# KKKSQJ/DeepLearning

Hardware: NVIDIA H100
Metric: images/sec (ResNet-50 training step) (higher is better)
Workload: dtype bf16

## Files before the change

deeplearning_b200/csrc/abi_conv.cu:

```cuda
#include <string.h>
#include "../../include/b200cls.h"
#include "conv_gemm.cuh"
#include "conv1x1_stream.cuh"
#include "conv_tap64.cuh"
#include "host_utils.h"
#include "wgrad_gemm.cuh"

using namespace b200;

namespace {

constexpr uint32_t kFwdDescLbo = 16, kFwdDescSbo = 1024;
constexpr uint32_t kWgDescLbo = 8192, kWgDescSbo = 1024, kWgDescKstep = 2048;

struct Box3 {
  int b1, b2, b3;
};

Box3 choose_box(long long d1, long long d2, long long d3, int P) {
  Box3 best{P, 1, 1};
  double best_cost = -1;
  for (int b1 = 1; b1 <= P; b1 <<= 1) {
    for (int b2 = 1; b1 * b2 <= P; b2 <<= 1) {
      const int b3 = P / (b1 * b2);
// ... 245 lines not shown
  B200_CHECK_CUDA(launch_pdl(conv_tap64_kernel<kStats>, dim3(grid), dim3(384), kTap64SmemBytes, st, q));
  B200_LAUNCHED();
  return OK;
}

template <int BLOCK_N>
int launch_conv_gemm(const ConvGemmParams& p, cudaStream_t st) {
  const int tiles = p.tiles1 * p.tiles2 * p.tiles3 * p.n_tiles;
  const int grid = conv_grid(tiles, p.n_tiles, p.stats != nullptr);
  B200_REQUIRE(grid > 0, "conv_gemm: %d channel blocks exceed the SM count (BN statistics need grid %% n_tiles == 0)", p.n_tiles);
  ConvGemmParams q = p;
  q.desc_lbo = kFwdDescLbo;
  q.desc_sbo = kFwdDescSbo;
  if constexpr (BLOCK_N == 64) {
    if (tap64_ok(p)) return p.stats != nullptr ? launch_tap64<true>(q, grid, st) : launch_tap64<false>(q, grid, st);
  }
  switch (epilogue_flags(p)) {
#define B200_EPI_CASE(F) \
  case (F):              \
    return launch_conv_gemm_epi<BLOCK_N, (F)>(q, grid, st);
    B200_EPI_LIST(B200_EPI_CASE)
#undef B200_EPI_CASE
    default:
      return launch_conv_gemm_epi<BLOCK_N, kEpiGeneric>(q, grid, st);
  }
}


bool stream_ok(long long pixels, int K, int N) {
  return (K == 64 || K == 128 || K == 256) && N % 256 == 0 && pixels % 128 == 0 && pixels / 128 < (1LL << 30);
}
int stream_grid(long long pixels, int N) {
  const int n_tiles = N / 256;
  const long long items = pixels / 128 * n_tiles;
  int grid = items < device_sm_count() ? static_cast<int>(items) : device_sm_count();
  return grid / n_tiles * n_tiles;
}

template <int KB, int MODE>
int launch_stream(const StreamParams& q, int grid, cudaStream_t st) {
  using Cfg = StreamCfg<KB, MODE>;
  static bool configured = false;
  if (!configured) {
    B200_CHECK_CUDA(cudaFuncSetAttribute(conv1x1_stream_kernel<KB, MODE>, cudaFuncAttributeMaxDynamicSharedMemorySize,
                                         Cfg::SMEM_BYTES));
    configured = true;
  }
  B200_CHECK_CUDA(launch_pdl(conv1x1_stream_kernel<KB, MODE>, dim3(grid), dim3(Cfg::THREADS), Cfg::SMEM_BYTES, st, q));
  B200_LAUNCHED();
  return OK;
}

int run_stream(int mode, const void* a, const void* w, void* out, const void* res, const void* mask, const float* scale,
               const float* shift, float* stats, long long pixels, int K, int N, cudaStream_t st) {
  StreamParams q;
  memset(&q, 0, sizeof(q));
  int rc;
  if ((rc = encode_matrix(&q.a_map, a, K, pixels, 128))) return rc;
  if ((rc = encode_matrix(&q.b_map, w, K, N, 256))) return rc;
  if ((rc = encode_matrix(&q.out_map, out, N, pixels, 16))) return rc;
  if (res != nullptr && (rc = encode_matrix(&q.res_map, res, N, pixels, 16))) return rc;
  if (mask != nullptr && (rc = encode_matrix(&q.mask_map, mask, N, pixels, 16))) return rc;
  q.m_tiles = static_cast<int>(pixels / 128);
  q.n_tiles = N / 256;
  q.N = N;
  q.scale = scale, q.shift = shift, q.stats = stats;
  const int grid = stream_grid(pixels, N);
  if (mode == kStreamAffine)
    return K == 64 ? launch_stream<1, kStreamAffine>(q, grid, st)
                   : (K == 128 ? launch_stream<2, kStreamAffine>(q, grid, st) : launch_stream<4, kStreamAffine>(q, grid, st));
  if (mode == kStreamBnRelu)
    return K == 64 ? launch_stream<1, kStreamBnRelu>(q, grid, st)
                   : (K == 128 ? launch_stream<2, kStreamBnRelu>(q, grid, st) : launch_stream<4, kStreamBnRelu>(q, grid, st));
  return K == 64 ? launch_stream<1, kStreamMask>(q, grid, st)
                 : (K == 128 ? launch_stream<2, kStreamMask>(q, grid, st) : launch_stream<4, kStreamMask>(q, grid, st));
}

int dispatch_conv_gemm(ConvGemmParams& p, int N, cudaStream_t st) {
  if (N <= 64) return launch_conv_gemm<64>(p, st);
  return launch_conv_gemm<128>(p, st);
}
int block_n_for(int N) { return N <= 64 ? 64 : 128; }

template <int BLOCK_NG, bool kGrouped = false>
int launch_wgrad(const WgradParams& p, cudaStream_t st) {
  using Cfg = WgradCfg<BLOCK_NG>;
  static bool configured = false;
  if (!configured) {
    if constexpr (kGrouped) {
      B200_CHECK_CUDA(cudaFuncSetAttribute(wgrad_gemm_kernel<BLOCK_NG, false, true>,
                                           cudaFuncAttributeMaxDynamicSharedMemorySize, Cfg::SMEM_BYTES));
    } else {
      B200_CHECK_CUDA(cudaFuncSetAttribute(wgrad_gemm_kernel<BLOCK_NG, false>, cudaFuncAttributeMaxDynamicSharedMemorySize,
                                           Cfg::SMEM_BYTES));
      B200_CHECK_CUDA(cudaFuncSetAttribute(wgrad_gemm_kernel<BLOCK_NG, true>, cudaFuncAttributeMaxDynamicSharedMemorySize,
                                           Cfg::SMEM_BYTES));
    }
    configured = true;
  }
  const int items = p.mg_tiles * p.ng_tiles * p.num_taps * p.splits;
  const int grid = items < device_sm_count() ? items : device_sm_count();
  WgradParams q = p;
  q.desc_lbo = kWgDescLbo;
  q.desc_sbo = kWgDescSbo;
  q.desc_kstep = kWgDescKstep;
  if constexpr (kGrouped)
    B200_CHECK_CUDA(launch_pdl(wgrad_gemm_kernel<BLOCK_NG, false, true>, dim3(grid), dim3(kWgradThreads), Cfg::SMEM_BYTES, st, q));
  else if (q.bias_partial != nullptr)
    B200_CHECK_CUDA(launch_pdl(wgrad_gemm_kernel<BLOCK_NG, true>, dim3(grid), dim3(kWgradThreads), Cfg::SMEM_BYTES, st, q));
  else
    B200_CHECK_CUDA(launch_pdl(wgrad_gemm_kernel<BLOCK_NG, false>, dim3(grid), dim3(kWgradThreads), Cfg::SMEM_BYTES, st, q));
  B200_LAUNCHED();
  return OK;
}

int launch_wgrad_reduce(const float* partial, float* dw, int splits, int Cout, int Cin, int taps, int accumulate,
                        cudaStream_t st, const float* bias_partial = nullptr, float* bias_out = nullptr) {
  const long long total = static_cast<long long>(Cout) * Cin * taps;
  if (Cin % 8 == 0 && (reinterpret_cast<uintptr_t>(partial) & 15) == 0) {
    int chunk = taps == 1 ? 256 : 64;
    while (chunk > 16 && chunk / 2 >= Cin) chunk /= 2;
    while (chunk > 16 && static_cast<long long>(Cout) * ((Cin + chunk - 1) / chunk) < 2ll * device_sm_count()) chunk /= 2;
    const int SL = splits < 8 ? splits : 8;
    const size_t smem = static_cast<size_t>(SL) * taps * chunk * sizeof(float);
    if (smem <= 48 * 1024 && Cout <= 65535 * 32) {
      dim3 grid(Cout, (Cin + chunk - 1) / chunk);
      B200_CHECK_CUDA(launch_pdl(wgrad_reduce_rows_kernel, dim3(grid), dim3(256), smem, st, partial, dw, splits, Cout, Cin, taps, chunk, SL, accumulate, bias_partial, bias_out));
      return OK;
    }
  }
  int blocks = static_cast<int>((total + 255) / 256);
  if (blocks > device_sm_count() * 8) blocks = device_sm_count() * 8;
  B200_CHECK_CUDA(launch_pdl(wgrad_reduce_flat_kernel, dim3(blocks), dim3(256), 0, st, partial, dw, splits, Cout, Cin, taps, accumulate, bias_partial, bias_out));
  return OK;
}

struct WgradPlan {
  int block_ng, mg_tiles, ng_tiles, taps;
  int merge_atoms;
  Box3 box;
  int tiles1, tiles2, tiles3, kb_total, splits, kb_per_split;
  int Ho, Wo;
};

WgradPlan plan_wgrad_geom(long long d1, long long d2, long long d3, int Cin, int Cout, int taps, bool grouped = false) {
  WgradPlan pl;
  pl.taps = taps;
  pl.Ho = static_cast<int>(d2), pl.Wo = static_cast<int>(d1);
  pl.block_ng = Cin <= 64 ? 64 : (((Cin + 255) / 256) * 48 < ((Cin + 127) / 128) * 32 ? 256 : 128);
  pl.mg_tiles = (Cout + 127) / 128;
  pl.ng_tiles = (Cin + pl.block_ng - 1) / pl.block_ng;
  pl.merge_atoms = 0;
  if (grouped) {
    pl.block_ng = 384;
    pl.ng_tiles = 1;
  } else if (Cin == 64 && taps > 1 && (taps % 4 == 0 || taps % 3 == 0)) {
    pl.merge_atoms = 1;
    pl.block_ng = taps % 4 == 0 ? 256 : 192;
    pl.ng_tiles = taps * 64 / pl.block_ng;
  }
  pl.box = choose_box(d1, d2, d3, 64);
  pl.tiles1 = static_cast<int>((d1 + pl.box.b1 - 1) / pl.box.b1);
  pl.tiles2 = static_cast<int>((d2 + pl.box.b2 - 1) / pl.box.b2);
  pl.tiles3 = static_cast<int>((d3 + pl.box.b3 - 1) / pl.box.b3);
  pl.kb_total = pl.tiles1 * pl.tiles2 * pl.tiles3;
  const int items_per_split = pl.mg_tiles * pl.ng_tiles * (pl.merge_atoms ? 1 : (grouped ? pl.taps / 3 : pl.taps));
  const int sms = device_sm_count();
  const double t_kb = pl.block_ng >= 256 ? 0.45 : (pl.block_ng == 192 ? 0.36 : (pl.block_ng == 128 ? 0.30 : 0.25));
  const double part_us = static_cast<double>(Cout) * Cin * taps * 4.0 * 2.0 / 3.0e6;
  const int max_splits = pl.kb_total / 4 > 0 ? pl.kb_total / 4 : 1;
  int splits = 1;
  double best = 1e30;
  for (int s = 1; s <= max_splits; ++s) {
    const int kps = (pl.kb_total + s - 1) / s;
    const int s2 = (pl.kb_total + kps - 1) / kps;
    if (s2 != s) continue;
    const int waves = (items_per_split * s + sms - 1) / sms;
    if (waves > 2 && items_per_split <= sms) continue;
    const double cost = waves * (kps * t_kb + 2.0) + s * part_us;
    if (cost < best) best = cost, splits = s;
    if (waves > 4 && s > 8) break;
  }
  pl.kb_per_split = (pl.kb_total + splits - 1) / splits;
  pl.splits = (pl.kb_total + pl.kb_per_split - 1) / pl.kb_per_split;
  return pl;
}

WgradPlan plan_wgrad(int B, int H, int W, int Cin, int Cout, int ksize, int stride, bool grouped = false) {
  const Dims3 d = out_dims(B, H, W, ksize, stride);
  WgradPlan pl = plan_wgrad_geom(d.d1, d.d2, d.d3, Cin, Cout, ksize * ksize, grouped);
  pl.Ho = out_dim(H, ksize, stride), pl.Wo = out_dim(W, ksize, stride);
  return pl;
}

size_t wgrad_bytes(const WgradPlan& pl, int Cout, int Cin) {
  return static_cast<size_t>(pl.splits) * Cout * pl.taps * Cin * sizeof(float);
}

WgradParams wgrad_params(const WgradPlan& pl, int Cout, int Cin, void* workspace) {
  WgradParams p;
  memset(&p, 0, sizeof(p));
  p.num_taps = pl.merge_atoms ? 1 : pl.taps;
  p.merge_atoms = pl.merge_atoms;
  p.n_cols = pl.merge_atoms ? pl.taps * Cin : Cin;
  p.Cout = Cout, p.Cin = Cin;
  p.mg_tiles = pl.mg_tiles, p.ng_tiles = pl.ng_tiles;
  p.tiles1 = pl.tiles1, p.tiles2 = pl.tiles2, p.tiles3 = pl.tiles3;
  p.box1 = pl.box.b1, p.box2 = pl.box.b2, p.box3 = pl.box.b3;
  p.splits = pl.splits, p.kb_per_split = pl.kb_per_split, p.kb_total = pl.kb_total;
  p.ld_partial = static_cast<long long>(pl.taps) * Cin;
  p.partial = static_cast<float*>(workspace);
  return p;
}

int setup_wgrad_maps(WgradParams& p, const WgradPlan& pl, const void* dy, const void* x, int B, int H, int W, int Cin,
                     int Cout, int ksize, int stride) {
  int rc;
  if ((rc = encode_view(&p.dy_map, act_view(dy, B, pl.Ho, pl.Wo, Cout, ksize == 1 && stride == 1), pl.box))) return rc;
  return encode_taps(p, p.x_maps, x, B, H, W, Cin, ksize, stride, pl.box);
}

View stem_s2d_view(const void* z, int B, int Ho, int Wo) {
  const int Hz = Ho + 3, Wz = Wo + 3;
  View v;
  v.base = z;
  v.dims[0] = 64, v.dims[1] = Wo, v.dims[2] = Hz, v.dims[3] = B;
  v.strides[0] = 1, v.strides[1] = 16, v.strides[2] = static_cast<uint64_t>(Wz) * 16;
  v.strides[3] = static_cast<uint64_t>(Hz) * Wz * 16;
  return v;
}

}

extern "C" {

static int fwd_stats_rows(int B, int H, int W, int Cout, int ksize, int stride, int BN) {
  const Dims3 d = out_dims(B, H, W, ksize, stride);
  const Box3 bx = choose_box(d.d1, d.d2, d.d3, 128);
  const long long m_tiles = ((d.d1 + bx.b1 - 1) / bx.b1) * ((d.d2 + bx.b2 - 1) / bx.b2) * ((d.d3 + bx.b3 - 1) / bx.b3);
  const int n_tiles = (Cout + BN - 1) / BN;
  const long long tiles = m_tiles * n_tiles;
  const int grid = conv_grid(tiles > (1 << 30) ? (1 << 30) : static_cast<int>(tiles), n_tiles, true);
  return grid / n_tiles * (BN == 64 ? 8 : 4);
}

int b200_conv2d_fwd_stats_rows(int B, int H, int W, int Cout, int ksize, int stride) {
  return fwd_stats_rows(B, H, W, Cout, ksize, stride, block_n_for(Cout));
}

static int conv_fwd(const void* x, const void* w, void* y, int B, int H, int W, int Cin, int Cout, int ksize, int stride,
                    float* stats, const float* bias, int act, const void* residual, float* out_f32, long long ld_out,
                    const float* bn_scale, const float* bn_shift, int y_f32, int Cg, void* stream) {
  B200_REQUIRE(ksize == 1 || ksize == 3 || (ksize == 2 && stride == 2), "conv2d_fwd: ksize %d / stride %d unsupported", ksize, stride);
  B200_REQUIRE(stride == 1 || stride == 2, "conv2d_fwd: stride %d unsupported (1 or 2)", stride);
  B200_REQUIRE(Cin % 8 == 0 && Cout % 8 == 0, "conv2d_fwd: Cin=%d / Cout=%d must be multiples of 8", Cin, Cout);
  B200_REQUIRE(B > 0 && H > 0 && W > 0, "conv2d_fwd: empty input");
  B200_REQUIRE(stride == 1 || (H >= 2 && W >= 2), "conv2d_fwd: stride-2 needs H,W >= 2");
  B200_REQUIRE(out_f32 == nullptr || (ksize == 1 && stride == 1), "conv2d_fwd: fp32 output only for 1x1/s1");
  B200_REQUIRE((bn_scale == nullptr) == (bn_shift == nullptr), "conv2d_fwd: bn_scale and bn_shift go together");
  B200_REQUIRE(bn_scale == nullptr || (Cout % 64 == 0 && bias == nullptr && stats == nullptr && out_f32 == nullptr && act <= 1 && !y_f32),
               "conv2d_fwd + folded BN: Cout=%d must be a multiple of 64, no bias / statistics / fp32 output", Cout);
  cudaStream_t st = static_cast<cudaStream_t>(stream);
  const int Ho = out_dim(H, ksize, stride), Wo = out_dim(W, ksize, stride);
  ConvGemmParams p;
  memset(&p, 0, sizeof(p));
  int rc;
  View dv = act_view(y, B, Ho, Wo, Cout, ksize == 1 && stride == 1);
  if (out_f32 != nullptr) dv.base = nullptr;
// ... 115 lines not shown
int b200_conv2d_dgrad(const void* dy, const void* wd, void* dx, int B, int H, int W, int Cin, int Cout, int ksize,
                      int stride, const void* residual, const b200_bn_mask_t* bn_mask, void* stream) {
  return conv_dgrad(dy, wd, dx, B, H, W, Cin, Cout, ksize, stride, residual, bn_mask, 0, stream);
}

int b200_gemm_ex(const b200_view_t* a, const b200_view_t* out, const b200_gemm_args_t* g, void* stream) {
  B200_REQUIRE(a != nullptr && out != nullptr && g != nullptr && g->w != nullptr, "gemm_ex: null argument");
  B200_REQUIRE(g->N % 8 == 0 && g->K % 8 == 0, "gemm_ex: N=%d / K=%d must be multiples of 8", g->N, g->K);
  for (int i = 0; i < 3; ++i)
    B200_REQUIRE(a->dim[i] == out->dim[i] && a->dim[i] > 0, "gemm_ex: a/out pixel extents differ in dim %d", i);
  B200_REQUIRE(!(g->aux_out != nullptr && g->out_f32), "gemm_ex: aux_out needs a bf16 primary output");
  B200_REQUIRE(!(g->stats != nullptr && g->out_f32), "gemm_ex: stats need a bf16 output");
  auto to_view = [](const b200_view_t* v, int C) {
    View r;
    r.base = v->base;
    r.dims[0] = C;
    r.strides[0] = 1;
    for (int i = 0; i < 3; ++i) {
      r.dims[i + 1] = static_cast<uint64_t>(v->dim[i]);
      r.strides[i + 1] = static_cast<uint64_t>(v->stride[i]);
    }
    return r;
  };
  ConvGemmParams p;
  memset(&p, 0, sizeof(p));
  int rc;
  View dv = to_view(out, g->N);
  View auxv;
  if (g->aux_out) auxv = to_view(g->aux_out, g->N);
  if ((rc = setup_output(p, dv, g->N, g->out_f32, g->aux_out ? &auxv : nullptr))) return rc;
  const Box3 bx = box_of(p);
  if ((rc = encode_view(&p.a_maps[0], to_view(a, g->K), bx))) return rc;
  for (int i = 1; i < 4; ++i) p.a_maps[i] = p.a_maps[0];
  p.num_taps = 1;
  p.k_per_tap = g->K;
  p.k_blocks_per_tap = (g->K + 63) / 64;
  if ((rc = encode_matrix(&p.b_map, g->w, g->K, g->N, block_n_for(g->N)))) return rc;
  p.stats = g->stats;
  p.bias = g->bias;
  p.colscale = g->colscale;
  p.act = g->act;
  if (g->residual) {
    p.residual = g->residual->base;
    p.res_f32 = g->residual_f32;
    p.rs1 = g->residual->stride[0], p.rs2 = g->residual->stride[1], p.rs3 = g->residual->stride[2];
  }
  if (g->rowscale != nullptr) {
    B200_REQUIRE(g->rows_per_sample > 0, "gemm_ex: rowscale needs rows_per_sample > 0");
    p.rowscale = g->rowscale;
    p.rows_per_sample = g->rows_per_sample;
  }
  if (g->act == B200_ACT_GELU_GRAD) {
    B200_REQUIRE(g->aux_in != nullptr, "gemm_ex: B200_ACT_GELU_GRAD needs aux_in");
    p.aux_in = static_cast<const __nv_bfloat16*>(g->aux_in->base);
    p.as1 = g->aux_in->stride[0], p.as2 = g->aux_in->stride[1], p.as3 = g->aux_in->stride[2];
  }
  return dispatch_conv_gemm(p, g->N, static_cast<cudaStream_t>(stream));
}

int b200_conv2d_wgrad_splits(int B, int H, int W, int Cin, int Cout, int ksize, int stride) {
  return plan_wgrad(B, H, W, Cin, Cout, ksize, stride).splits;
}

size_t b200_conv2d_wgrad_workspace_bytes(int B, int H, int W, int Cin, int Cout, int ksize, int stride) {
  return wgrad_bytes(plan_wgrad(B, H, W, Cin, Cout, ksize, stride), Cout, Cin);
}

int b200_conv2d_wgrad(const void* dy, const void* x, float* dw, void* workspace, size_t workspace_bytes, int B, int H,
                      int W, int Cin, int Cout, int ksize, int stride, int accumulate, float* bias_partial, float* bias_out,
                      void* stream) {
  B200_REQUIRE(ksize == 1 || ksize == 3 || (ksize == 2 && stride == 2), "conv2d_wgrad: ksize %d / stride %d unsupported", ksize, stride);
  B200_REQUIRE(stride == 1 || stride == 2, "conv2d_wgrad: stride %d unsupported", stride);
  B200_REQUIRE(Cin % 8 == 0 && Cout % 8 == 0, "conv2d_wgrad: Cin=%d / Cout=%d must be multiples of 8", Cin, Cout);
  B200_REQUIRE(bias_out == nullptr || bias_partial != nullptr, "conv2d_wgrad: bias_out needs bias_partial");
  cudaStream_t st = static_cast<cudaStream_t>(stream);
  const WgradPlan pl = plan_wgrad(B, H, W, Cin, Cout, ksize, stride);
  const size_t need = wgrad_bytes(pl, Cout, Cin);
  B200_REQUIRE(workspace != nullptr && workspace_bytes >= need, "conv2d_wgrad: workspace too small (%zu < %zu)",
               workspace_bytes, need);
  WgradParams p = wgrad_params(pl, Cout, Cin, workspace);
  p.bias_partial = bias_partial;
  int rc;
  if ((rc = setup_wgrad_maps(p, pl, dy, x, B, H, W, Cin, Cout, ksize, stride))) return rc;
  if (pl.block_ng == 64)
    rc = launch_wgrad<64>(p, st);
  else if (pl.block_ng == 128)
    rc = launch_wgrad<128>(p, st);
  else if (pl.block_ng == 192)
    rc = launch_wgrad<192>(p, st);
  else
    rc = launch_wgrad<256>(p, st);
  if (rc) return rc;
  if ((rc = launch_wgrad_reduce(p.partial, dw, pl.splits, Cout, Cin, pl.taps, accumulate, st, bias_partial, bias_out))) return rc;
  B200_LAUNCHED();
  return OK;
}

int b200_stem_s2d_conv_fwd(const void* z, const void* w, void* y, float* stats, int B, int Ho, int Wo, void* stream) {
  B200_REQUIRE(B > 0 && Ho > 0 && Wo > 0, "stem_s2d_conv_fwd: empty output");
  cudaStream_t st = static_cast<cudaStream_t>(stream);
  const int Cout = 64;
  ConvGemmParams p;
  memset(&p, 0, sizeof(p));
  int rc;
  if ((rc = setup_output(p, make_view(y, B, Ho, Wo, Cout, 1, 0, 0), Cout, 0, nullptr))) return rc;
  const Box3 bx = box_of(p);
  p.k_per_tap = 64;
  p.k_blocks_per_tap = 1;
  p.num_taps = 4;
  if ((rc = encode_view(&p.a_maps[0], stem_s2d_view(z, B, Ho, Wo), bx))) return rc;
  for (int i = 1; i < 4; ++i) p.a_maps[i] = p.a_maps[0];
  for (int ky = 0; ky < 4; ++ky) {
    p.tap_map[ky] = 0, p.tap_o1[ky] = 0, p.tap_o2[ky] = static_cast<int8_t>(ky), p.tap_w[ky] = static_cast<int8_t>(ky);
  }
  if ((rc = encode_matrix(&p.b_map, w, 256, Cout, 64))) return rc;
  p.stats = stats;
  return dispatch_conv_gemm(p, Cout, st);
}

size_t b200_stem_s2d_conv_wgrad_workspace_bytes(int B, int Ho, int Wo) {
  return wgrad_bytes(plan_wgrad_geom(Wo, Ho, B, 64, 64, 4), 64, 64);
}

int b200_stem_s2d_conv_wgrad(const void* dy, const void* z, float* g, void* workspace, size_t workspace_bytes, int B, int Ho,
                             int Wo, void* stream) {
  cudaStream_t st = static_cast<cudaStream_t>(stream);
  const int Cout = 64, Cin = 64, taps = 4;
  const WgradPlan pl = plan_wgrad_geom(Wo, Ho, B, Cin, Cout, taps);
  const size_t need = wgrad_bytes(pl, Cout, Cin);
  B200_REQUIRE(workspace != nullptr && workspace_bytes >= need, "stem_s2d_conv_wgrad: workspace too small (%zu < %zu)",
               workspace_bytes, need);
  WgradParams p = wgrad_params(pl, Cout, Cin, workspace);
  int rc;
  if ((rc = encode_view(&p.dy_map, make_view(dy, B, Ho, Wo, Cout, 1, 0, 0), pl.box))) return rc;
  if ((rc = encode_view(&p.x_maps[0], stem_s2d_view(z, B, Ho, Wo), pl.box))) return rc;
  for (int i = 1; i < 4; ++i) p.x_maps[i] = p.x_maps[0];
  for (int ky = 0; ky < 4; ++ky) p.tap_map[ky] = 0, p.tap_o1[ky] = 0, p.tap_o2[ky] = static_cast<int8_t>(ky);
  if ((rc = launch_wgrad<256>(p, st))) return rc;
  if ((rc = launch_wgrad_reduce(p.partial, g, pl.splits, Cout, Cin, taps, 0, st))) return rc;
  B200_LAUNCHED();
  return OK;
}


int b200_conv1x1_bn_act_fwd(const void* x, const void* w, const float* scale, const float* shift, const void* residual,
                            void* y, long long pixels, int Cin, int Cout, int relu, void* stream) {
  B200_REQUIRE(pixels > 0 && Cin % 64 == 0 && Cout % 64 == 0, "conv1x1_bn_act_fwd: Cin=%d / Cout=%d must be multiples of 64", Cin, Cout);
  B200_REQUIRE(scale != nullptr && shift != nullptr && residual != nullptr && relu == 1,
               "conv1x1_bn_act_fwd: implemented for relu(bn(conv) + residual)");
  if (stream_ok(pixels, Cin, Cout))
    return run_stream(kStreamBnRelu, x, w, y, residual, nullptr, scale, shift, nullptr, pixels, Cin, Cout,
                      static_cast<cudaStream_t>(stream));
  ConvGemmParams p;
  memset(&p, 0, sizeof(p));
  int rc;
  View dv = make_flat_view(y, pixels, Cout);
  if ((rc = setup_output(p, dv, Cout, 0, nullptr))) return rc;
  const Box3 bx = box_of(p);
  p.k_per_tap = Cin;
  p.k_blocks_per_tap = Cin / 64;
  p.num_taps = 1;
  if ((rc = encode_view(&p.a_maps[0], make_flat_view(x, pixels, Cin), bx))) return rc;
  for (int i = 1; i < 4; ++i) p.a_maps[i] = p.a_maps[0];
  if ((rc = encode_matrix(&p.b_map, w, Cin, Cout, block_n_for(Cout)))) return rc;
  p.affine = 1;
  p.colscale = scale;
  p.bias = shift;
  p.act = 1;
  p.residual = residual;
  p.rs1 = static_cast<long long>(dv.strides[1]);
  p.rs2 = static_cast<long long>(dv.strides[2]);
  p.rs3 = static_cast<long long>(dv.strides[3]);
  return dispatch_conv_gemm(p, Cout, static_cast<cudaStream_t>(stream));
}

int b200_conv1x1_bn_fwd(const void* x, const void* w, const float* scale, const float* shift, void* y, long long pixels,
                        int Cin, int Cout, void* stream) {
  B200_REQUIRE(pixels > 0 && Cin % 64 == 0 && Cout % 64 == 0, "conv1x1_bn_fwd: Cin=%d / Cout=%d must be multiples of 64", Cin, Cout);
  B200_REQUIRE(scale != nullptr && shift != nullptr, "conv1x1_bn_fwd: scale / shift required");
  if (stream_ok(pixels, Cin, Cout))
    return run_stream(kStreamAffine, x, w, y, nullptr, nullptr, scale, shift, nullptr, pixels, Cin, Cout,
                      static_cast<cudaStream_t>(stream));
  return conv_fwd(x, w, y, 1, 1, static_cast<int>(pixels), Cin, Cout, 1, 1, nullptr, nullptr, 0, nullptr, nullptr, 0, scale,
                  shift, 0, 0, stream);
}

int b200_conv1x1_dgrad_masked_stats_rows(long long pixels, int Cin, int Cout) {
  if (stream_ok(pixels, Cout, Cin)) return stream_grid(pixels, Cin) / (Cin / 256) * 4;
  return b200_conv2d_fwd_stats_rows(1, 1, static_cast<int>(pixels), Cin, 1, 1);
}

int b200_conv1x1_dgrad_masked(const void* dy, const void* wd, void* dx, long long pixels, int Cin, int Cout,
                              const void* residual, const void* mask_src, float* stats, void* stream) {
  B200_REQUIRE(pixels > 0 && Cin % 64 == 0 && Cout % 64 == 0, "conv1x1_dgrad_masked: Cin=%d / Cout=%d must be multiples of 64", Cin, Cout);
  B200_REQUIRE(residual != nullptr && mask_src != nullptr && stats != nullptr, "conv1x1_dgrad_masked: residual, mask and stats are required");
  if (stream_ok(pixels, Cout, Cin))
    return run_stream(kStreamMask, dy, wd, dx, residual, mask_src, nullptr, nullptr, stats, pixels, Cout, Cin,
                      static_cast<cudaStream_t>(stream));
  ConvGemmParams p;
  memset(&p, 0, sizeof(p));
  int rc;
  View dv = make_flat_view(dx, pixels, Cin);
  if ((rc = setup_output(p, dv, Cin, 0, nullptr))) return rc;
  const Box3 bx = box_of(p);
  p.k_per_tap = Cout;
  p.k_blocks_per_tap = Cout / 64;
  p.num_taps = 1;
  if ((rc = encode_view(&p.a_maps[0], make_flat_view(dy, pixels, Cout), bx))) return rc;
  for (int i = 1; i < 4; ++i) p.a_maps[i] = p.a_maps[0];
  if ((rc = encode_matrix(&p.b_map, wd, Cout, Cin, block_n_for(Cin)))) return rc;
  p.residual = residual;
  p.rs1 = static_cast<long long>(dv.strides[1]);
  p.rs2 = static_cast<long long>(dv.strides[2]);
  p.rs3 = static_cast<long long>(dv.strides[3]);
  p.mask_in = static_cast<const __nv_bfloat16*>(mask_src);
  p.ms1 = p.rs1, p.ms2 = p.rs2, p.ms3 = p.rs3;
  p.stats = stats;
  return dispatch_conv_gemm(p, Cin, static_cast<cudaStream_t>(stream));
}

int b200_gemm_dual(const void* a0, int K0, const void* a1, int K1, const void* wcat, const float* bias, void* out,
// ... 90 lines not shown
```

deeplearning_b200/csrc/wgrad_gemm.cuh:

```cuda
#pragma once
#include "common.cuh"
#include "conv_gemm.cuh"
#include "conv1x1_stream.cuh"

namespace b200 {

struct alignas(64) WgradParams {
  CUtensorMap dy_map;
  CUtensorMap x_maps[4];
  int num_taps;
  int merge_atoms;
  int n_cols;
  int Cout, Cin;
  int mg_tiles, ng_tiles;
  int tiles1, tiles2, tiles3;
  int box1, box2, box3;
  int splits, kb_per_split, kb_total;
  long long ld_partial;
  int8_t tap_map[kMaxTaps];
  int8_t tap_o1[kMaxTaps];
  int8_t tap_o2[kMaxTaps];
  float* partial;
  uint32_t desc_lbo, desc_sbo, desc_kstep;
  float* bias_partial;
};

template <int BLOCK_NG>
struct WgradCfg {
  static constexpr int BLOCK_K = 64;
  static constexpr int A_BYTES = 2 * 64 * 128;
  static constexpr int B_BYTES = (BLOCK_NG / 64) * 64 * 128;
  static constexpr int STAGE_BYTES = A_BYTES + B_BYTES;
  static constexpr int STAGES = BLOCK_NG == 384 ? 3 : (BLOCK_NG == 256 ? 4 : (BLOCK_NG == 192 ? 5 : (BLOCK_NG == 128 ? 6 : 8)));
  static constexpr int BAR_BYTES = 256;
  static constexpr int SMEM_BYTES = STAGES * STAGE_BYTES + BAR_BYTES + 1024;
  static_assert(SMEM_BYTES <= 227 * 1024, "shared memory of one H100 block");
};
constexpr int kWgradThreads = 384;

template <int BLOCK_NG, bool kBias = false, bool kGrouped = false>
__global__ void __launch_bounds__(kWgradThreads, 1) wgrad_gemm_kernel(const __grid_constant__ WgradParams p) {
  static_assert(!kGrouped || (BLOCK_NG == 384 && !kBias), "grouped mode: two warpgroups x three 64-column taps");
  using Cfg = WgradCfg<BLOCK_NG>;
  constexpr int NW = kGrouped ? BLOCK_NG / 2 : BLOCK_NG;
  constexpr int STAGES = Cfg::STAGES;
  extern __shared__ uint8_t smem_raw[];
  uint8_t* smem = reinterpret_cast<uint8_t*>((reinterpret_cast<uintptr_t>(smem_raw) + 1023) & ~uintptr_t(1023));
  uint64_t* bars = reinterpret_cast<uint64_t*>(smem + STAGES * Cfg::STAGE_BYTES);
  uint64_t* full_bar = bars;
  uint64_t* empty_bar = bars + STAGES;
  __shared__ float bias_red[2][16][64];

  const int warp_idx = threadIdx.x >> 5;
  const int lane = threadIdx.x & 31;
  const int items_per_split = p.mg_tiles * p.ng_tiles * p.num_taps;
  const int num_items = items_per_split * p.splits;

  if (warp_idx == 0 && lane == 0) {
    tma_prefetch_desc(&p.dy_map);
    for (int i = 0; i < 4; ++i) tma_prefetch_desc(&p.x_maps[i]);
    for (int i = 0; i < STAGES; ++i) {
      mbar_init(&full_bar[i], 1);
      mbar_init(&empty_bar[i], kBias ? 8 : 2);
    }
    fence_mbar_init();
  }
  __syncthreads();
  pdl_wait();

  if (warp_idx < 4) {
    setmaxnreg_dec<40>();
    if (warp_idx == 0 && lane == 0) {
      int stage = 0;
      uint32_t phase = 0;
      for (int item = blockIdx.x; item < num_items; item += gridDim.x) {
        const int split = item / items_per_split;
        int r = item - split * items_per_split;
        const int tap = r % p.num_taps;
        r /= p.num_taps;
        const int ng = r % p.ng_tiles;
        const int mg = r / p.ng_tiles;
        const int kb0 = split * p.kb_per_split;
        const int kb1 = min(p.kb_total, kb0 + p.kb_per_split);
        const CUtensorMap* xm[BLOCK_NG / 64];
        int ch0[BLOCK_NG / 64], o1[BLOCK_NG / 64], o2[BLOCK_NG / 64];
#pragma unroll
        for (int j = 0; j < BLOCK_NG / 64; ++j) {
          int tp = tap, ca = ng * (BLOCK_NG / 64) + j;
          if constexpr (kGrouped) {
            tp = tap * 3 + j % 3;
            ca = mg * 2 + j / 3;
          } else if (p.merge_atoms) {
            tp = ca / p.merge_atoms;
            ca -= tp * p.merge_atoms;
          }
          xm[j] = &p.x_maps[p.tap_map[tp]];
          ch0[j] = ca * 64;
          o1[j] = p.tap_o1[tp], o2[j] = p.tap_o2[tp];
        }
        for (int kb = kb0; kb < kb1; ++kb) {
          const int t1 = kb % p.tiles1;
          const int t2 = (kb / p.tiles1) % p.tiles2;
          const int t3 = kb / (p.tiles1 * p.tiles2);
          const int c1 = t1 * p.box1, c2 = t2 * p.box2, c3 = t3 * p.box3;
          mbar_wait(&empty_bar[stage], phase ^ 1);
          uint8_t* a_dst = smem + stage * Cfg::STAGE_BYTES;
          uint8_t* b_dst = a_dst + Cfg::A_BYTES;
          mbar_expect_tx(&full_bar[stage], Cfg::STAGE_BYTES);
          tma_load_4d(a_dst, &p.dy_map, &full_bar[stage], mg * 128, c1, c2, c3);
          tma_load_4d(a_dst + 8192, &p.dy_map, &full_bar[stage], mg * 128 + 64, c1, c2, c3);
#pragma unroll
          for (int j = 0; j < BLOCK_NG / 64; ++j)
            tma_load_4d(b_dst + j * 8192, xm[j], &full_bar[stage], ch0[j], c1 + o1[j], c2 + o2[j], c3);
          if (++stage == STAGES) {
            stage = 0;
            phase ^= 1;
          }
        }
      }
    }
  } else {
    setmaxnreg_inc<232>();
    const int wg = (warp_idx >> 2) - 1;
    const bool leader = (threadIdx.x & 127) == 0;
    const uint64_t desc_a0 = make_smem_desc_sw128(smem_u32(smem) + wg * 8192, p.desc_lbo, p.desc_sbo);
    const uint64_t desc_b0 =
        make_smem_desc_sw128(smem_u32(smem) + Cfg::A_BYTES + (kGrouped ? wg * NW * 128 : 0), p.desc_lbo, p.desc_sbo);
    const uint64_t kstep = p.desc_kstep >> 4;
    const int t = threadIdx.x & 127;
    const int frow = 64 * wg + 16 * (t >> 5) + ((t & 31) >> 2);
    const int fcol = 2 * (t & 3);
    int stage = 0;
    uint32_t phase = 0;
    for (int item = blockIdx.x; item < num_items; item += gridDim.x) {
      const int split = item / items_per_split;
      int r = item - split * items_per_split;
      const int tap = r % p.num_taps;
      r /= p.num_taps;
      const int ng = r % p.ng_tiles;
      const int mg = r / p.ng_tiles;
      const int kb0 = split * p.kb_per_split;
      const int kb1 = min(p.kb_total, kb0 + p.kb_per_split);
      const bool summed = kBias && ng == 0 && tap == 0;
      const int cc = t & 7, rg = t >> 3;
      float bsum[8] = {0.f, 0.f, 0.f, 0.f, 0.f, 0.f, 0.f, 0.f};
      float acc[NW / 2];
#pragma unroll
      for (int i = 0; i < NW / 2; ++i) acc[i] = 0.f;
      int prev = -1;
      for (int kb = kb0; kb < kb1; ++kb) {
        mbar_wait(&full_bar[stage], phase);
        wgmma_fence();
        const uint64_t soff = static_cast<uint64_t>(stage) * (Cfg::STAGE_BYTES >> 4);
        const uint64_t da = desc_a0 + soff, db = desc_b0 + soff;
#pragma unroll
        for (int k = 0; k < 4; ++k) Wgmma<NW, 1, 1>::mma(acc, da + k * kstep, db + k * kstep, 1u);
        wgmma_commit();
        if (summed) {
          const uint32_t base = smem_u32(smem + stage * Cfg::STAGE_BYTES) + wg * 8192;
#pragma unroll
          for (int i = 0; i < 4; ++i) {
            const int r = rg * 4 + i;
            float f[8];
            unpack8(lds128(base + r * 128 + ((static_cast<uint32_t>(cc) ^ static_cast<uint32_t>(r & 7)) << 4)), f);
#pragma unroll
            for (int j = 0; j < 8; ++j) bsum[j] += f[j];
          }
        }
        wgmma_wait<1>();
        if constexpr (kBias) {
          __syncwarp();
          if (prev >= 0 && lane == 0) mbar_arrive(&empty_bar[prev]);
        } else {
          if (prev >= 0 && leader) mbar_arrive(&empty_bar[prev]);
        }
        prev = stage;
        if (++stage == STAGES) {
          stage = 0;
          phase ^= 1;
        }
      }
      wgmma_wait<0>();
      wgmma_reg_fence(acc);
      if constexpr (kBias) {
        __syncwarp();
        if (lane == 0) mbar_arrive(&empty_bar[prev]);
      } else {
        if (leader) mbar_arrive(&empty_bar[prev]);
      }
      if (summed) {
        named_bar_sync(1 + wg, 128);
#pragma unroll
        for (int j = 0; j < 8; ++j) bias_red[wg][rg][cc * 8 + j] = bsum[j];
        named_bar_sync(1 + wg, 128);
        if (t < 64) {
          float tot = 0.f;
#pragma unroll
          for (int g2 = 0; g2 < 16; ++g2) tot += bias_red[wg][g2][t];
          const int cout = mg * 128 + wg * 64 + t;
          if (cout < p.Cout) {
            p.bias_partial[(static_cast<long long>(split) * 2) * p.Cout + cout] = tot;
            p.bias_partial[(static_cast<long long>(split) * 2 + 1) * p.Cout + cout] = 0.f;
          }
        }
      }
      const int ncol = p.n_cols - ng * BLOCK_NG;
#pragma unroll
      for (int h = 0; h < 2; ++h) {
        const int cout = mg * 128 + frow + 8 * h;
        if (cout < p.Cout) {
          float* out_row = p.partial + (static_cast<long long>(split) * p.Cout + cout) * p.ld_partial +
                           static_cast<long long>(tap) * p.Cin + ng * BLOCK_NG;
#pragma unroll
          for (int j = 0; j < NW / 8; ++j)
            if (8 * j + fcol < ncol)
              *reinterpret_cast<float2*>(out_row + 8 * j + fcol) = make_float2(acc[4 * j + 2 * h], acc[4 * j + 2 * h + 1]);
        }
      }
    }
  }
}

__global__ void __launch_bounds__(256) wgrad_reduce_rows_kernel(const float* __restrict__ partial, float* __restrict__ grad,
                                                                int splits, int Cout, int Cin, int taps, int chunk, int SL,
                                                                int accumulate, const float* __restrict__ bias_partial,
                                                                float* __restrict__ bias_out) {
  pdl_wait();
  extern __shared__ float4 rows_sm4[];
  const int cout = blockIdx.x;
  if (bias_out != nullptr && blockIdx.y == 0 && threadIdx.x == 0) {
    float s = 0.f;
    for (int k = 0; k < splits; ++k) s += bias_partial[static_cast<long long>(k) * 2 * Cout + cout];
    bias_out[cout] = s;
  }
  const int c0 = blockIdx.y * chunk;
  const int cw = min(chunk, Cin - c0);
  const int vpt = cw >> 2;
  const int nvec = taps * vpt;
  const long long slice4 = static_cast<long long>(Cout) * taps * Cin / 4;
  const float4* row4 = reinterpret_cast<const float4*>(partial + static_cast<long long>(cout) * taps * Cin + c0);
  const int cin4 = Cin >> 2;
  for (int w = threadIdx.x; w < nvec * SL; w += blockDim.x) {
    const int sl = w / nvec;
    const int v = w - sl * nvec;
    const int tap = v / vpt;
    const int cv = v - tap * vpt;
    const float4* src = row4 + tap * cin4 + cv;
    float4 a = make_float4(0.f, 0.f, 0.f, 0.f), b = a;
    int k = sl;
    for (; k + SL < splits; k += 2 * SL) {
      const float4 x = __ldcs(src + k * slice4);
      const float4 y = __ldcs(src + (k + SL) * slice4);
      a.x += x.x, a.y += x.y, a.z += x.z, a.w += x.w;
      b.x += y.x, b.y += y.y, b.z += y.z, b.w += y.w;
    }
    if (k < splits) {
      const float4 x = __ldcs(src + k * slice4);
      a.x += x.x, a.y += x.y, a.z += x.z, a.w += x.w;
    }
    rows_sm4[w] = make_float4(a.x + b.x, a.y + b.y, a.z + b.z, a.w + b.w);
  }
  __syncthreads();
  const float* sm = reinterpret_cast<const float*>(rows_sm4);
  float* out = grad + (static_cast<long long>(cout) * Cin + c0) * taps;
  for (int e = threadIdx.x; e < cw * taps; e += blockDim.x) {
    const int cin = e / taps;
    const int tap = e - cin * taps;
    float s = 0.f;
    for (int sl = 0; sl < SL; ++sl) s += sm[(sl * nvec) * 4 + tap * cw + cin];
    out[e] = accumulate ? out[e] + s : s;
  }
}

__global__ void wgrad_reduce_flat_kernel(const float* __restrict__ partial, float* __restrict__ grad, int splits, int Cout,
                                    int Cin, int taps, int accumulate, const float* __restrict__ bias_partial,
                                    float* __restrict__ bias_out) {
  pdl_wait();
  const long long total = static_cast<long long>(Cout) * Cin * taps;
  const long long slice = total;
  if (bias_out != nullptr) {
    for (int cout = blockIdx.x * blockDim.x + threadIdx.x; cout < Cout; cout += gridDim.x * blockDim.x) {
      float s = 0.f;
      for (int k = 0; k < splits; ++k) s += bias_partial[static_cast<long long>(k) * 2 * Cout + cout];
      bias_out[cout] = s;
    }
  }
  for (long long i = blockIdx.x * static_cast<long long>(blockDim.x) + threadIdx.x; i < total;
       i += static_cast<long long>(gridDim.x) * blockDim.x) {
    const int cin = static_cast<int>(i % Cin);
    const long long t = i / Cin;
    const int tap = static_cast<int>(t % taps);
    const int cout = static_cast<int>(t / taps);
    float s = 0.f;
    for (int k = 0; k < splits; ++k) s += partial[k * slice + i];
    const long long o = (static_cast<long long>(cout) * Cin + cin) * taps + tap;
    grad[o] = accumulate ? grad[o] + s : s;
  }
}
// ... 21 lines not shown
```

Before: 8779.

## Split wgrad tile across warpgroups by columns when Cout fits in 64

For weight-gradient GEMMs with Cout <= 64, the block loads only 64 rows of dy and splits the N (input-channel) columns between the two consumer warpgroups instead of splitting rows. Previously half the 128-row A tile was padding for such layers, which wasted TMA bandwidth, shared memory and tensor-core issue. The smaller stage size allows more pipeline stages. When a warpgroup's column slice straddles a 64-column swizzle atom, the MMA is split into two wgmma calls, which adds code complexity and a risk of descriptor errors.

```diff
diff --git a/deeplearning_b200/csrc/abi_conv.cu b/deeplearning_b200/csrc/abi_conv.cu
--- a/deeplearning_b200/csrc/abi_conv.cu
+++ b/deeplearning_b200/csrc/abi_conv.cu
@@ -351,19 +351,19 @@
 }
 int block_n_for(int N) { return N <= 64 ? 64 : 128; }
 
-template <int BLOCK_NG, bool kGrouped = false>
+template <int BLOCK_NG, bool kGrouped = false, bool kNSplit = false>
 int launch_wgrad(const WgradParams& p, cudaStream_t st) {
-  using Cfg = WgradCfg<BLOCK_NG>;
+  using Cfg = WgradCfg<BLOCK_NG, kNSplit>;
   static bool configured = false;
   if (!configured) {
     if constexpr (kGrouped) {
       B200_CHECK_CUDA(cudaFuncSetAttribute(wgrad_gemm_kernel<BLOCK_NG, false, true>,
                                            cudaFuncAttributeMaxDynamicSharedMemorySize, Cfg::SMEM_BYTES));
     } else {
-      B200_CHECK_CUDA(cudaFuncSetAttribute(wgrad_gemm_kernel<BLOCK_NG, false>, cudaFuncAttributeMaxDynamicSharedMemorySize,
-                                           Cfg::SMEM_BYTES));
-      B200_CHECK_CUDA(cudaFuncSetAttribute(wgrad_gemm_kernel<BLOCK_NG, true>, cudaFuncAttributeMaxDynamicSharedMemorySize,
-                                           Cfg::SMEM_BYTES));
+      B200_CHECK_CUDA(cudaFuncSetAttribute(wgrad_gemm_kernel<BLOCK_NG, false, false, kNSplit>,
+                                           cudaFuncAttributeMaxDynamicSharedMemorySize, Cfg::SMEM_BYTES));
+      B200_CHECK_CUDA(cudaFuncSetAttribute(wgrad_gemm_kernel<BLOCK_NG, true, false, kNSplit>,
+                                           cudaFuncAttributeMaxDynamicSharedMemorySize, Cfg::SMEM_BYTES));
     }
     configured = true;
   }
@@ -376,9 +376,11 @@
   if constexpr (kGrouped)
     B200_CHECK_CUDA(launch_pdl(wgrad_gemm_kernel<BLOCK_NG, false, true>, dim3(grid), dim3(kWgradThreads), Cfg::SMEM_BYTES, st, q));
   else if (q.bias_partial != nullptr)
-    B200_CHECK_CUDA(launch_pdl(wgrad_gemm_kernel<BLOCK_NG, true>, dim3(grid), dim3(kWgradThreads), Cfg::SMEM_BYTES, st, q));
+    B200_CHECK_CUDA(launch_pdl(wgrad_gemm_kernel<BLOCK_NG, true, false, kNSplit>, dim3(grid), dim3(kWgradThreads),
+                               Cfg::SMEM_BYTES, st, q));
   else
-    B200_CHECK_CUDA(launch_pdl(wgrad_gemm_kernel<BLOCK_NG, false>, dim3(grid), dim3(kWgradThreads), Cfg::SMEM_BYTES, st, q));
+    B200_CHECK_CUDA(launch_pdl(wgrad_gemm_kernel<BLOCK_NG, false, false, kNSplit>, dim3(grid), dim3(kWgradThreads),
+                               Cfg::SMEM_BYTES, st, q));
   B200_LAUNCHED();
   return OK;
 }
@@ -407,6 +409,7 @@
 struct WgradPlan {
   int block_ng, mg_tiles, ng_tiles, taps;
   int merge_atoms;
+  bool nsplit;
   Box3 box;
   int tiles1, tiles2, tiles3, kb_total, splits, kb_per_split;
   int Ho, Wo;
@@ -428,6 +431,7 @@
     pl.block_ng = taps % 4 == 0 ? 256 : 192;
     pl.ng_tiles = taps * 64 / pl.block_ng;
   }
+  pl.nsplit = !grouped && Cout <= 64;
   pl.box = choose_box(d1, d2, d3, 64);
   pl.tiles1 = static_cast<int>((d1 + pl.box.b1 - 1) / pl.box.b1);
   pl.tiles2 = static_cast<int>((d2 + pl.box.b2 - 1) / pl.box.b2);
@@ -453,6 +457,19 @@
   pl.kb_per_split = (pl.kb_total + splits - 1) / splits;
   pl.splits = (pl.kb_total + pl.kb_per_split - 1) / pl.kb_per_split;
   return pl;
+}
+
+int launch_wgrad_plan(const WgradPlan& pl, const WgradParams& p, cudaStream_t st) {
+  if (pl.nsplit) {
+    if (pl.block_ng == 64) return launch_wgrad<64, false, true>(p, st);
+    if (pl.block_ng == 128) return launch_wgrad<128, false, true>(p, st);
+    if (pl.block_ng == 192) return launch_wgrad<192, false, true>(p, st);
+    return launch_wgrad<256, false, true>(p, st);
+  }
+  if (pl.block_ng == 64) return launch_wgrad<64>(p, st);
+  if (pl.block_ng == 128) return launch_wgrad<128>(p, st);
+  if (pl.block_ng == 192) return launch_wgrad<192>(p, st);
+  return launch_wgrad<256>(p, st);
 }
 
 WgradPlan plan_wgrad(int B, int H, int W, int Cin, int Cout, int ksize, int stride, bool grouped = false) {
@@ -734,15 +751,7 @@
   p.bias_partial = bias_partial;
   int rc;
   if ((rc = setup_wgrad_maps(p, pl, dy, x, B, H, W, Cin, Cout, ksize, stride))) return rc;
-  if (pl.block_ng == 64)
-    rc = launch_wgrad<64>(p, st);
-  else if (pl.block_ng == 128)
-    rc = launch_wgrad<128>(p, st);
-  else if (pl.block_ng == 192)
-    rc = launch_wgrad<192>(p, st);
-  else
-    rc = launch_wgrad<256>(p, st);
-  if (rc) return rc;
+  if ((rc = launch_wgrad_plan(pl, p, st))) return rc;
   if ((rc = launch_wgrad_reduce(p.partial, dw, pl.splits, Cout, Cin, pl.taps, accumulate, st, bias_partial, bias_out))) return rc;
   B200_LAUNCHED();
   return OK;
@@ -788,7 +797,7 @@
   if ((rc = encode_view(&p.x_maps[0], stem_s2d_view(z, B, Ho, Wo), pl.box))) return rc;
   for (int i = 1; i < 4; ++i) p.x_maps[i] = p.x_maps[0];
   for (int ky = 0; ky < 4; ++ky) p.tap_map[ky] = 0, p.tap_o1[ky] = 0, p.tap_o2[ky] = static_cast<int8_t>(ky);
-  if ((rc = launch_wgrad<256>(p, st))) return rc;
+  if ((rc = launch_wgrad_plan(pl, p, st))) return rc;
   if ((rc = launch_wgrad_reduce(p.partial, g, pl.splits, Cout, Cin, taps, 0, st))) return rc;
   B200_LAUNCHED();
   return OK;
diff --git a/deeplearning_b200/csrc/wgrad_gemm.cuh b/deeplearning_b200/csrc/wgrad_gemm.cuh
--- a/deeplearning_b200/csrc/wgrad_gemm.cuh
+++ b/deeplearning_b200/csrc/wgrad_gemm.cuh
@@ -25,24 +25,28 @@
   float* bias_partial;
 };
 
-template <int BLOCK_NG>
+template <int BLOCK_NG, bool kNSplit = false>
 struct WgradCfg {
   static constexpr int BLOCK_K = 64;
-  static constexpr int A_BYTES = 2 * 64 * 128;
+  static constexpr int ROWS = kNSplit ? 64 : 128;
+  static constexpr int A_BYTES = (ROWS / 64) * 64 * 128;
   static constexpr int B_BYTES = (BLOCK_NG / 64) * 64 * 128;
   static constexpr int STAGE_BYTES = A_BYTES + B_BYTES;
-  static constexpr int STAGES = BLOCK_NG == 384 ? 3 : (BLOCK_NG == 256 ? 4 : (BLOCK_NG == 192 ? 5 : (BLOCK_NG == 128 ? 6 : 8)));
   static constexpr int BAR_BYTES = 256;
+  static constexpr int NSPLIT_STAGES = (227 * 1024 - 8192 - 1024 - BAR_BYTES) / STAGE_BYTES;
+  static constexpr int STAGES = kNSplit ? (NSPLIT_STAGES < 8 ? NSPLIT_STAGES : 8)
+                                        : (BLOCK_NG == 384 ? 3 : (BLOCK_NG == 256 ? 4 : (BLOCK_NG == 192 ? 5 : (BLOCK_NG == 128 ? 6 : 8))));
   static constexpr int SMEM_BYTES = STAGES * STAGE_BYTES + BAR_BYTES + 1024;
   static_assert(SMEM_BYTES <= 227 * 1024, "shared memory of one H100 block");
 };
 constexpr int kWgradThreads = 384;
 
-template <int BLOCK_NG, bool kBias = false, bool kGrouped = false>
+template <int BLOCK_NG, bool kBias = false, bool kGrouped = false, bool kNSplit = false>
 __global__ void __launch_bounds__(kWgradThreads, 1) wgrad_gemm_kernel(const __grid_constant__ WgradParams p) {
-  static_assert(!kGrouped || (BLOCK_NG == 384 && !kBias), "grouped mode: two warpgroups x three 64-column taps");
-  using Cfg = WgradCfg<BLOCK_NG>;
-  constexpr int NW = kGrouped ? BLOCK_NG / 2 : BLOCK_NG;
+  static_assert(!kGrouped || (BLOCK_NG == 384 && !kBias && !kNSplit), "grouped mode: two warpgroups x three 64-column taps");
+  using Cfg = WgradCfg<BLOCK_NG, kNSplit>;
+  constexpr int NW = kGrouped || kNSplit ? BLOCK_NG / 2 : BLOCK_NG;
+  constexpr int NW1 = NW % 64 == 0 || NW % 64 + NW <= 64 ? NW : 64 - NW % 64;
   constexpr int STAGES = Cfg::STAGES;
   extern __shared__ uint8_t smem_raw[];
   uint8_t* smem = reinterpret_cast<uint8_t*>((reinterpret_cast<uintptr_t>(smem_raw) + 1023) & ~uintptr_t(1023));
@@ -107,8 +111,8 @@
           uint8_t* a_dst = smem + stage * Cfg::STAGE_BYTES;
           uint8_t* b_dst = a_dst + Cfg::A_BYTES;
           mbar_expect_tx(&full_bar[stage], Cfg::STAGE_BYTES);
-          tma_load_4d(a_dst, &p.dy_map, &full_bar[stage], mg * 128, c1, c2, c3);
-          tma_load_4d(a_dst + 8192, &p.dy_map, &full_bar[stage], mg * 128 + 64, c1, c2, c3);
+          tma_load_4d(a_dst, &p.dy_map, &full_bar[stage], mg * Cfg::ROWS, c1, c2, c3);
+          if constexpr (!kNSplit) tma_load_4d(a_dst + 8192, &p.dy_map, &full_bar[stage], mg * 128 + 64, c1, c2, c3);
 #pragma unroll
           for (int j = 0; j < BLOCK_NG / 64; ++j)
             tma_load_4d(b_dst + j * 8192, xm[j], &full_bar[stage], ch0[j], c1 + o1[j], c2 + o2[j], c3);
@@ -123,12 +127,15 @@
     setmaxnreg_inc<232>();
     const int wg = (warp_idx >> 2) - 1;
     const bool leader = (threadIdx.x & 127) == 0;
-    const uint64_t desc_a0 = make_smem_desc_sw128(smem_u32(smem) + wg * 8192, p.desc_lbo, p.desc_sbo);
-    const uint64_t desc_b0 =
-        make_smem_desc_sw128(smem_u32(smem) + Cfg::A_BYTES + (kGrouped ? wg * NW * 128 : 0), p.desc_lbo, p.desc_sbo);
+    const int wrow = kNSplit ? 0 : 64 * wg;
+    const int wcol = kNSplit ? NW * wg : 0;
+    const uint32_t bcol_off = kGrouped ? wg * NW * 128 : (wcol / 64) * 8192 + (wcol % 64) * 2;
+    const uint64_t desc_a0 = make_smem_desc_sw128(smem_u32(smem) + wrow * 128, p.desc_lbo, p.desc_sbo);
+    const uint64_t desc_b0 = make_smem_desc_sw128(smem_u32(smem) + Cfg::A_BYTES + bcol_off, p.desc_lbo, p.desc_sbo);
+    const uint64_t desc_b1 = desc_b0 + ((8192 - (wcol % 64) * 2) >> 4);
     const uint64_t kstep = p.desc_kstep >> 4;
     const int t = threadIdx.x & 127;
-    const int frow = 64 * wg + 16 * (t >> 5) + ((t & 31) >> 2);
+    const int frow = wrow + 16 * (t >> 5) + ((t & 31) >> 2);
     const int fcol = 2 * (t & 3);
     int stage = 0;
     uint32_t phase = 0;
@@ -141,7 +148,7 @@
       const int mg = r / p.ng_tiles;
       const int kb0 = split * p.kb_per_split;
       const int kb1 = min(p.kb_total, kb0 + p.kb_per_split);
-      const bool summed = kBias && ng == 0 && tap == 0;
+      const bool summed = kBias && ng == 0 && tap == 0 && !(kNSplit && wg == 1);
       const int cc = t & 7, rg = t >> 3;
       float bsum[8] = {0.f, 0.f, 0.f, 0.f, 0.f, 0.f, 0.f, 0.f};
       float acc[NW / 2];
@@ -153,8 +160,19 @@
         wgmma_fence();
         const uint64_t soff = static_cast<uint64_t>(stage) * (Cfg::STAGE_BYTES >> 4);
         const uint64_t da = desc_a0 + soff, db = desc_b0 + soff;
-#pragma unroll
-        for (int k = 0; k < 4; ++k) Wgmma<NW, 1, 1>::mma(acc, da + k * kstep, db + k * kstep, 1u);
+        if (NW1 == NW || wg == 0) {
+#pragma unroll
+          for (int k = 0; k < 4; ++k) Wgmma<NW, 1, 1>::mma(acc, da + k * kstep, db + k * kstep, 1u);
+        } else if constexpr (NW1 != NW) {
+          float(&acc_lo)[NW1 / 2] = *reinterpret_cast<float(*)[NW1 / 2]>(acc);
+          float(&acc_hi)[(NW - NW1) / 2] = *reinterpret_cast<float(*)[(NW - NW1) / 2]>(acc + NW1 / 2);
+          const uint64_t db1 = desc_b1 + soff;
+#pragma unroll
+          for (int k = 0; k < 4; ++k) {
+            Wgmma<NW1, 1, 1>::mma(acc_lo, da + k * kstep, db + k * kstep, 1u);
+            Wgmma<NW - NW1, 1, 1>::mma(acc_hi, da + k * kstep, db1 + k * kstep, 1u);
+          }
+        }
         wgmma_commit();
         if (summed) {
           const uint32_t base = smem_u32(smem + stage * Cfg::STAGE_BYTES) + wg * 8192;
@@ -197,7 +215,7 @@
           float tot = 0.f;
 #pragma unroll
           for (int g2 = 0; g2 < 16; ++g2) tot += bias_red[wg][g2][t];
-          const int cout = mg * 128 + wg * 64 + t;
+          const int cout = mg * Cfg::ROWS + wrow + t;
           if (cout < p.Cout) {
             p.bias_partial[(static_cast<long long>(split) * 2) * p.Cout + cout] = tot;
             p.bias_partial[(static_cast<long long>(split) * 2 + 1) * p.Cout + cout] = 0.f;
@@ -207,13 +225,13 @@
       const int ncol = p.n_cols - ng * BLOCK_NG;
 #pragma unroll
       for (int h = 0; h < 2; ++h) {
-        const int cout = mg * 128 + frow + 8 * h;
+        const int cout = mg * Cfg::ROWS + frow + 8 * h;
         if (cout < p.Cout) {
           float* out_row = p.partial + (static_cast<long long>(split) * p.Cout + cout) * p.ld_partial +
-                           static_cast<long long>(tap) * p.Cin + ng * BLOCK_NG;
+                           static_cast<long long>(tap) * p.Cin + ng * BLOCK_NG + wcol;
 #pragma unroll
           for (int j = 0; j < NW / 8; ++j)
-            if (8 * j + fcol < ncol)
+            if (wcol + 8 * j + fcol < ncol)
               *reinterpret_cast<float2*>(out_row + 8 * j + fcol) = make_float2(acc[4 * j + 2 * h], acc[4 * j + 2 * h + 1]);
         }
       }
```

New measurement: 8887 (median of 6 runs). +1.2%, better.
